# rkhosrowshahi/MO-VAE

Hardware: AMD Instinct MI355X
Metric: training images/sec (higher is better)
Workload: dtype f32

## Files before the change

include/movae.h:

```cpp
#ifndef MOVAE_H
#define MOVAE_H

#include <stddef.h>
#include <stdint.h>

#ifdef __cplusplus
extern "C" {
#endif

typedef void* movae_stream_t;

enum movae_act { MOVAE_ACT_NONE = 0, MOVAE_ACT_LRELU = 1, MOVAE_ACT_RELU = 2, MOVAE_ACT_TANH = 3, MOVAE_ACT_SIGMOID = 4 };
enum movae_recon { MOVAE_RECON_MSE = 0, MOVAE_RECON_BCE = 1, MOVAE_RECON_L1 = 2, MOVAE_RECON_SMOOTH_L1 = 3 };
enum movae_mgda_norm { MOVAE_MGDA_NONE = 0, MOVAE_MGDA_L2 = 1, MOVAE_MGDA_LOSS = 2, MOVAE_MGDA_LOSS_PLUS = 3 };
enum movae_upgrad_norm { MOVAE_UPGRAD_TRACE = 0, MOVAE_UPGRAD_MIN_L2 = 1, MOVAE_UPGRAD_COSINE = 2 };
enum movae_amtl_scale { MOVAE_AMTL_MIN = 0, MOVAE_AMTL_MEDIAN = 1, MOVAE_AMTL_RMSE = 2 };

int movae_version(void);
const char* movae_last_error(void);

int movae_nchw_to_nhwc(const float* src, float* dst, int n, int c, int h, int w, movae_stream_t stream);
int movae_nhwc_to_nchw(const float* src, float* dst, int n, int c, int h, int w, movae_stream_t stream);

int movae_conv2d_fwd(const float* x, const float* w, const float* bias, float* y,
// ... 135 lines not shown
int movae_vq_nearest_fwd_mse(const float* x, const float* e, float* q, int64_t* idx, float* sse, int32_t* used_count, float* mse2,
                             int rows, int k, int d, void* ws, size_t ws_bytes, movae_stream_t stream);
size_t movae_vq_bwd_ws_bytes(int rows, int k, int d);
int movae_vq_bwd(const float* x, const float* q, const int64_t* idx, const float* dq, const float* gc, const float* ge,
                 float* dx, float* de, int rows, int k, int d, void* ws, size_t ws_bytes, movae_stream_t stream);

#define MOVAE_MAX_K 8
size_t movae_gram_ws_bytes(int k, size_t m);
int movae_gram(const float* J, size_t ldj, int k, size_t m, float* G, void* ws, size_t ws_bytes, movae_stream_t stream);
int movae_weights_upgrad(const float* G, int k, float norm_eps, float reg_eps, const float* pref, float* w, movae_stream_t stream);
int movae_weights_upgrad_norm(const float* G, int k, int norm_mode, float norm_eps, float reg_eps, const float* pref, float* w,
                              movae_stream_t stream);
int movae_gram_upgrad(const float* J, size_t ldj, int k, size_t m, float* G, int norm_mode, float norm_eps, float reg_eps,
                      const float* pref, float* w, int dual, void* ws, size_t ws_bytes, movae_stream_t stream);
int movae_weights_mgda(const float* G, int k, int norm, const float* losses, float epsilon, int max_iters,
                       float* w, int32_t* info, movae_stream_t stream);
int movae_weights_mgda_stable(const float* G, int k, int norm, const float* losses, float epsilon, int max_iters,
                              float min_eigenvalue, float* w, int32_t* info, movae_stream_t stream);
int movae_weights_amtl(const float* G, int k, int scale_mode, const float* pref, float* w, movae_stream_t stream);
int movae_weights_dualproj(const float* G, int k, float norm_eps, float reg_eps, const float* pref, float* w, movae_stream_t stream);
int movae_weights_pcgrad(const float* G, int k, const int32_t* perm, float* w, movae_stream_t stream);
int movae_weights_imtlg(const float* G, int k, float* w, movae_stream_t stream);
int movae_weights_cagrad(const float* G, int k, float c, float norm_eps, float* w, movae_stream_t stream);
int movae_weights_const(int k, float value, float* w, movae_stream_t stream);
int movae_combine(const float* J, size_t ldj, int k, size_t m, const float* w, float* g, int accumulate, movae_stream_t stream);
int movae_gd_similarity(const float* J, size_t ldj, int k, size_t m, const float* w, float* out,
                        void* ws, size_t ws_bytes, movae_stream_t stream);

int movae_adam_step(float* p, const float* g, float* m, float* v, size_t n, float lr, float beta1, float beta2,
                    float eps, float weight_decay, int decoupled_wd, int step, movae_stream_t stream);
int movae_adam_multi(int n_tensors, float* const* p, const float* const* g, float* const* m, float* const* v,
                     const size_t* numel, float lr, float beta1, float beta2, float eps, float weight_decay,
                     int decoupled_wd, int step, float* hyper_dev, movae_stream_t stream);
int movae_clip_grad_norm_multi(int n_tensors, float* const* g, const size_t* numel, float max_norm, float* total_sumsq_dev,
                               void* ws, size_t ws_bytes, movae_stream_t stream);
int movae_sumsq(const float* x, size_t n, float* out, void* ws, size_t ws_bytes, movae_stream_t stream);
int movae_scale_by_clip(float* g, size_t n, const float* sumsq_dev, float max_norm, movae_stream_t stream);

#define MOVAE_DTYPE_F32 0
#define MOVAE_DTYPE_BF16 1
int movae_set_compute_dtype(int dtype);

int movae_reduce_defer(int on);
int movae_reduce_flush(void);
int movae_reduce_defer_stats(long long* out3, int reset);
long long movae_reduce_defer_max_bytes(long long bytes);

int movae_bench_main_kernel_only(int on);
const char* movae_bench_last_kernel(void);
int movae_bench_force_split(int s);
int movae_bench_kgemm_bn_fin(int mode);
int movae_bench_force_kgemm(int mode);

typedef struct movae_fuse {
    const float* in_scale;
    const float* in_shift;
    float in_slope;
    float* stats;
    size_t stats_cap;
    int stats_parts;
    const float* bn_y;
    const float* bn_scale;
    const float* bn_shift;
    float bn_slope;
    float* bn_part;
    size_t bn_cap;
// ... 109 lines not shown
```

mo-vae_amd/_lib.py:

```python
import ctypes as C
import os
import threading

import torch

HERE = os.path.dirname(os.path.abspath(__file__))
LIB_PATH = os.path.join(HERE, "libmovae_hip.so")

ACT = {"none": 0, None: 0, "lrelu": 1, "relu": 2, "tanh": 3, "sigmoid": 4}
RECON = {"mse": 0, "bce": 1, "l1": 2, "smooth_l1": 3}
UPGRAD_NORM = {"trace": 0, "min_l2": 1, "cosine": 2}
EDGE_MATCH = {"mag": 0, "signed_mse": 1, "maxnorm": 2, "angle": 3, "masked": 4, "cosine": 5}
MGDA_NORM = {"none": 0, "l2": 1, "loss": 2, "loss+": 3}
AMTL_SCALE = {"min": 0, "median": 1, "rmse": 2}
MAX_K = 8

_p, _i, _f, _z, _l = C.c_void_p, C.c_int, C.c_float, C.c_size_t, C.c_long

class MovaeFuse(C.Structure):
    _fields_ = [("in_scale", C.c_void_p), ("in_shift", C.c_void_p), ("in_slope", C.c_float), ("stats", C.c_void_p),
                ("stats_cap", C.c_size_t), ("stats_parts", C.c_int),
                ("bn_y", C.c_void_p), ("bn_scale", C.c_void_p), ("bn_shift", C.c_void_p), ("bn_slope", C.c_float), ("bn_part", C.c_void_p),
                ("bn_cap", C.c_size_t), ("bn_ppg", C.c_int),
                ("ep_act_y", C.c_void_p), ("ep_act", C.c_int), ("ep_slope", C.c_float), ("ep_act_done", C.c_int),
# ... 51 lines not shown
    "movae_sphere_latents_fwd": ([_p, _p, _p, _p, _i, _f, _i, _p, _i, _i, _i, _f, _f, _f, _f, _f, _f] + [_p] * 6 + [_p], _i),
    "movae_sphere_latents_bwd": ([_p] * 9 + [_i, _i, _f, _p], _i),
    "movae_sphere_losses_ws_bytes": ([_z, _i], _z),
    "movae_sphere_losses_fwd": ([_p, _p, _p, _p, _z, _p, _p, _i, _i, _f, _f, _f, _f, _f, _p, _p, _z, _p], _i),
    "movae_sphere_losses_bwd": ([_p, _p, _p, _p, _z, _p, _p, _i, _i, _f, _f, _f, _f, _f] + [_p] * 8 + [_p], _i),
    "movae_tc_decomp_fwd": ([_p] * 7 + [_i, _i, _p, _z, _p], _i),
    "movae_tc_decomp_bwd": ([_p] * 10 + [_i, _i, _p], _i),
    "movae_edge_weights": ([_p, _p, _p, _i, _i, _i, _i, _p, _z, _p], _i),
    "movae_edge_weighted_mse_fwd": ([_p, _p, _p, _p, _p, _i, _i, _i, _i, _f, _p, _z, _p], _i),
    "movae_edge_weighted_mse_bwd": ([_p, _p, _p, _p, _p, _p, _i, _i, _i, _i, _f, _p], _i),
    "movae_edge_match_fwd": ([_p, _p, _p, _i, _i, _i, _i, _f, _i, _p, _p, _z, _p], _i),
    "movae_edge_match_bwd": ([_p, _p, _p, _p, _p, _p, _i, _i, _i, _i, _f, _i, _p, _p], _i),
    "movae_vq_nearest_fwd": ([_p] * 6 + [_i, _i, _i, _p, _z, _p], _i),
    "movae_vq_nearest_fwd_mse": ([_p] * 7 + [_i, _i, _i, _p, _z, _p], _i),
    "movae_vq_bwd_ws_bytes": ([_i, _i, _i], _z),
    "movae_vq_bwd": ([_p] * 8 + [_i, _i, _i, _p, _z, _p], _i),
    "movae_gram_ws_bytes": ([_i, _z], _z),
    "movae_gram": ([_p, _z, _i, _z, _p, _p, _z, _p], _i),
    "movae_weights_upgrad": ([_p, _i, _f, _f, _p, _p, _p], _i),
    "movae_weights_upgrad_norm": ([_p, _i, _i, _f, _f, _p, _p, _p], _i),
    "movae_gram_upgrad": ([_p, _z, _i, _z, _p, _i, _f, _f, _p, _p, _i, _p, _z, _p], _i),
    "movae_weights_mgda": ([_p, _i, _i, _p, _f, _i, _p, _p, _p], _i),
    "movae_weights_mgda_stable": ([_p, _i, _i, _p, _f, _i, _f, _p, _p, _p], _i),
    "movae_weights_amtl": ([_p, _i, _i, _p, _p, _p], _i),
    "movae_weights_dualproj": ([_p, _i, _f, _f, _p, _p, _p], _i),
    "movae_weights_pcgrad": ([_p, _i, _p, _p, _p], _i),
    "movae_weights_imtlg": ([_p, _i, _p, _p], _i),
    "movae_weights_cagrad": ([_p, _i, _f, _f, _p, _p], _i),
    "movae_weights_const": ([_i, _f, _p, _p], _i),
    "movae_combine": ([_p, _z, _i, _z, _p, _p, _i, _p], _i),
    "movae_gd_similarity": ([_p, _z, _i, _z, _p, _p, _p, _z, _p], _i),
    "movae_adam_step": ([_p, _p, _p, _p, _z, _f, _f, _f, _f, _f, _i, _i, _p], _i),
    "movae_adam_multi": ([_i, _p, _p, _p, _p, _p, _f, _f, _f, _f, _f, _i, _i, _p, _p], _i),
    "movae_clip_grad_norm_multi": ([_i, _p, _p, _f, _p, _p, _z, _p], _i),
    "movae_sumsq": ([_p, _z, _p, _p, _z, _p], _i),
    "movae_scale_by_clip": ([_p, _z, _p, _f, _p], _i),
    "movae_conv2d_fwd_f": (_conv_fwd + [_p], _i),
    "movae_convT2d_fwd_f": (_conv_fwd + [_p], _i),
    "movae_conv2d_wgrad_grouped_f": ([_i] + _conv_wgrad + [_p], _i),
    "movae_convT2d_wgrad_grouped_f": ([_i] + _conv_wgrad + [_p], _i),
    "movae_conv2d_dgrad_wgrad_grouped_f": ([_i, _p, _p, _p, _p, _p, _p] + [_i] * 11 + [_i, _p, _z, _p, _p], _i),
    "movae_convT2d_dgrad_wgrad_grouped_f": ([_i, _p, _p, _p, _p, _p, _p] + [_i] * 11 + [_i, _p, _z, _p, _p], _i),
    "movae_conv2d_dgrad_f": (_conv_dgrad + [_p, _i], _i),
    "movae_convT2d_dgrad_f": (_conv_dgrad + [_p, _i], _i),
    "movae_bn_bwd_finalize": ([_p, _z, _i, _i, _i, _i, _p, _p, _p, _p, _p, _p, _i, _p], _i),
    "movae_bn_bwd_apply": ([_p, _p, _p, _p, _f, _p, _p, _i, _z, _i, _p], _i),
    "movae_linear_pair_fwd": ([_p, _p, _p, _p, _p, _p, _p, _i, _i, _i, _p], _i),
    "movae_linear_pair_bwd": ([_i, _p, _p, _p, _p, _p, _p, _p, _p, _p, _p, _i, _i, _i, _p], _i),
    "movae_bn_bwd_finalize_apply": ([_p, _z, _i, _i, _z, _i, _p, _p, _p, _p, _p, _p, _i, _p, _p, _p, _p, _f, _p, _p], _i),
    "movae_bn_finalize": ([_p, _z, _i, _i, _i, _p, _p, _f, _f, _p, _p, _p, _p, _p, _p, _p, _p], _i),
    "movae_bn_stats": ([_p, _i, _i, _p, _z, _p, _p], _i),
    "movae_scale_shift_act": ([_p, _p, _p, _p, _z, _i, _f, _p], _i),
    "movae_embedding_fwd": ([_p, _p, _p, _z, _i, _i, _p], _i),
    "movae_embedding_bwd": ([_p, _p, _p, _i, _i, _i, _p, _z, _p], _i),
    "movae_gated_residual_fwd": ([_p, _p, _p, _p, _z, _p], _i),
    "movae_gated_residual_bwd": ([_p, _p, _p, _p, _p, _z, _p], _i),
    "movae_mul": ([_p, _p, _p, _z, _p], _i),
    "movae_cross_entropy_ws_bytes": ([_z], _z),
    "movae_cross_entropy_fwd": ([_p, _p, _p, _p, _z, _i, _p, _z, _p], _i),
    "movae_cross_entropy_bwd": ([_p, _p, _p, _p, _p, _z, _i, _p], _i),
    "movae_causal_attn_fwd": ([_p, _p, _p, _l, _p, _p, _i, _i, _i, _i, _f, C.c_ulonglong, C.c_ulonglong, _p], _i),
    "movae_causal_attn_ws_bytes": ([_i, _i, _i], _z),
    "movae_causal_attn_bwd": ([_p, _p, _p, _l, _p, _p, _p, _p, _p, _p, _i, _i, _i, _i, _f, C.c_ulonglong, C.c_ulonglong, _p, _z, _p], _i),
    "movae_causal_attn_dropout_mask": ([_p, _i, _i, _f, C.c_ulonglong, C.c_ulonglong, _p], _i),
    "movae_attn_fwd": ([_p, _p, _p, _l, _p, _p, _p, _p, _i, _i, _i, _i, _f, _p], _i),
    "movae_attn_ws_bytes": ([_i, _i, _i], _z),
# ... 150 lines not shown
```

mo-vae_amd/aggregation.py:

```python
import os

import torch
import torch.nn as tnn

from . import _lib as L


def _st(t):
    return L.stream_ptr(t.device)


def _check_matrix(J):
    if J.dim() != 2:
        raise ValueError(f"Parameter `matrix` should be a tensor of dimension 2. Found `matrix.shape = {tuple(J.shape)}`.")
    if J.shape[0] > L.MAX_K:
        raise ValueError(f"at most {L.MAX_K} objectives are supported on device, got {J.shape[0]}")
    L.require_gpu(J)
    if J.dtype != torch.float32 or J.stride(1) != 1:
        raise ValueError("the Jacobian must be fp32 with unit column stride")


FUSE_GRAM = os.environ.get("MOVAE_FUSE_GRAM", "1") != "0"


# ... 33 lines not shown


class Weighting(tnn.Module):

    def forward(self, gramian):
        raise NotImplementedError


class _FromJacobian(tnn.Module):

    def __init__(self, gramian_weighting):
        super().__init__()
        self.gramian_weighting = gramian_weighting

    def forward(self, J):
        gw = self.gramian_weighting
        fused = getattr(gw, "from_jacobian", None)
        if fused is not None and FUSE_GRAM and not gw._forward_hooks and not gw._forward_pre_hooks:
            self.last_gramian, w = fused(J)
            return w
        self.last_gramian = compute_gramian(J)
        return gw(self.last_gramian)


class GramianWeightedAggregator(tnn.Module):
    def __init__(self, gramian_weighting):
        super().__init__()
        self.gramian_weighting = gramian_weighting
        self.weighting = _FromJacobian(gramian_weighting)

    def forward(self, J):
        w = self.weighting(J)
        return combine(J, w)


class UPGradWeighting(Weighting):

    def __init__(self, pref_vector=None, norm_eps=1e-4, reg_eps=1e-4, norm="trace"):
        super().__init__()
        self.pref_vector, self.norm_eps, self.reg_eps, self.norm = pref_vector, norm_eps, reg_eps, norm

    def _mode(self):
        return self.norm

    def forward(self, G):
        k = G.shape[0]
        w = torch.empty(k, dtype=torch.float32, device=G.device)
        pref = _pref_tensor(self.pref_vector, G.device)
        L.call("movae_weights_upgrad_norm", G.data_ptr(), k, L.UPGRAD_NORM[self._mode()], float(self.norm_eps),
               float(self.reg_eps), L.ptr(pref), w.data_ptr(), _st(G))
        return w

    def from_jacobian(self, J):
        _check_matrix(J)
        k, m = J.shape
        G = torch.empty((k, k), dtype=torch.float32, device=J.device)
        w = torch.empty(k, dtype=torch.float32, device=J.device)
        pref = _pref_tensor(self.pref_vector, J.device)
        ws = L.workspace(J.device)
        L.call("movae_gram_upgrad", J.data_ptr(), J.stride(0) if k > 1 else max(J.stride(0), m), k, m, G.data_ptr(),
               L.UPGRAD_NORM[self._mode()], float(self.norm_eps), float(self.reg_eps), L.ptr(pref), w.data_ptr(), 0, ws.data_ptr(),
               ws.numel(), _st(J))
        return G, w


class _PNUPGradWeighting(UPGradWeighting):
# ... 340 lines not shown
```

mo-vae_amd/autojac.py:

```python
import os

import torch

from . import ops

BATCHED_VJP = os.environ.get("MOVAE_BATCHED_VJP", "1") != "0"


def _leaf_tensors(roots, excluded=()):
    stop = {t.grad_fn for t in excluded if t.grad_fn is not None}
    seen, leaves, stack = set(), [], [t.grad_fn for t in roots if t.grad_fn is not None]
    while stack:
        fn = stack.pop()
        if fn is None or fn in seen or fn in stop:
            continue
        seen.add(fn)
        var = getattr(fn, "variable", None)
        if var is not None:
            if var.requires_grad:
                leaves.append(var)
            continue
        stack.extend(nf for nf, _ in fn.next_functions)
    out, ids = [], set()
    for v in leaves:
        if id(v) not in ids:
            ids.add(id(v))
            out.append(v)
    return out


def _mem_flat(t):
    if t.dim() == 4 and not t.is_contiguous():
# ... 222 lines not shown
                                     for i in range(len(per[0])))
                    if not isinstance(outs, tuple):
                        outs = (outs,)
                    need = [i for i, nd in enumerate(fn.needs_input_grad) if nd]
                    live = [j for j, (nf, _) in enumerate(edges) if nf is not None]
                    if len(need) != len(live):
                        raise NotImplementedError("cannot align backward outputs with graph edges")
                    aligned = [None] * len(edges)
                    for j, i in zip(live, need):
                        aligned[j] = outs[i] if i < len(outs) else None
                    outs = tuple(aligned)
                else:
                    per = []
                    for g in range(G):
                        r = fn(*[_group(a, g) for a in args])
                        per.append(r if isinstance(r, tuple) else (r,))
                    outs = tuple(None if all(per[g][i] is None for g in range(G)) else _restack([per[g][i] for g in range(G)])
                                 for i in range(len(per[0])))
            for i, (nf, nr) in enumerate(edges):
                if nf is None:
                    continue
                o = outs[i] if outs is not None and i < len(outs) else None
                if o is not None:
                    o = _fit_groups(o, _expected_shape(nf, nr), G)
                    slot = pending.setdefault(nf, {})
                    slot[nr] = _accumulate_stacked(slot.get(nr), o, G)
                deps[nf] -= 1
                if deps[nf] == 0:
                    ready.append(nf)
    finally:
        ops.GRAD_SINK_ROWS = None


def _aggregate_into_grads(jb, aggregator):
    g = aggregator(jb.J)
    for p, off in zip(jb.params, jb.offsets):
        _accumulate(p, _view_like(g[off: off + p.numel()], p))
    return g


class _MtlState:
    __slots__ = ("jb", "feat_diff", "feat_grads", "shared_params", "aggregator", "task_params", "device")


def mtl_backward_begin(losses, features, aggregator, tasks_params=None, shared_params=None):
    losses, features = list(losses), list(features)
    if len(losses) == 0:
        raise ValueError("`losses` cannot be empty")
    if len(features) == 0:
        raise ValueError("`features` cannot be empty.")
    if shared_params is None:
        shared_params = _leaf_tensors(features)
    if tasks_params is None:
        tasks_params = [_leaf_tensors([l], excluded=features) for l in losses]
    if len(tasks_params) != len(losses):
        raise ValueError("`losses` and `tasks_params` should have the same size.")
    st = _MtlState()
    st.shared_params = list(shared_params)
    st.aggregator = aggregator
    st.jb = JacobianBuffer.persistent(st.shared_params, len(losses), features[0].device)
    st.feat_diff = [f for f in features if f.requires_grad]
    st.feat_grads = []
    st.task_params = []
    cot = [torch.empty_strided((len(losses),) + tuple(f.shape), (f.numel(),) + tuple(f.stride()), dtype=f.dtype, device=f.device)
           if _dense(f) else None for f in st.feat_diff]
    for i, (loss, tp) in enumerate(zip(losses, tasks_params)):
        tp = list(tp)
        seed = _ones_like(loss) if loss.dim() == 0 and loss.dtype == torch.float32 else None
# ... 132 lines not shown
```

mo-vae_amd/csrc/agg.hip:

```cpp
#include "common.h"
#include <stdlib.h>

namespace {

constexpr int MAXK = MOVAE_MAX_K;
inline int gram_blocks(size_t m) {
    static const size_t cap = (size_t)env_long("MOVAE_GRAM_BLOCKS", 1024);
    size_t g = (m + 2047) / 2048;
    return (int)(g > cap ? cap : (g < 1 ? 1 : g));
}

template <int K, bool VEC>
__global__ __launch_bounds__(256) void gram_partial(const float* __restrict__ J, long ldj, long m, double* __restrict__ part) {
    constexpr int NP = K * (K + 1) / 2;
    double acc[NP];
#pragma unroll
    for (int q = 0; q < NP; ++q) acc[q] = 0.0;
    const long stride = (long)gridDim.x * blockDim.x;
    if (VEC) {
        const long nv = m / 4;
        for (long c = (long)blockIdx.x * blockDim.x + threadIdx.x; c < nv; c += stride) {
            f32x4 v[K];
#pragma unroll
            for (int i = 0; i < K; ++i) v[i] = reinterpret_cast<const f32x4*>(J + i * ldj)[c];
// ... 32 lines not shown
        if (threadIdx.x == 0) part[(long)blockIdx.x * NP + q] = s;
    }
}

__global__ __launch_bounds__(64) void gram_final(const double* __restrict__ part, int nblk, int K, float* __restrict__ G) {
    const int NP = K * (K + 1) / 2;
    const int q = blockIdx.x;
    double s = 0.0;
    for (int b = threadIdx.x; b < nblk; b += 64) s += part[(long)b * NP + q];
    s = wave_sum(s);
    if (threadIdx.x != 0) return;
    int i = 0, rem = q;
    while (rem >= K - i) {
        rem -= K - i;
        ++i;
    }
    const int j = i + rem;
    G[i * K + j] = (float)s;
    G[j * K + i] = (float)s;
}

template <int K, bool VEC>
__global__ __launch_bounds__(256) void combine_k(const float* __restrict__ J, long ldj, long m, const float* __restrict__ w,
                                                 float* __restrict__ g, int accumulate) {
    float wv[K];
#pragma unroll
    for (int i = 0; i < K; ++i) wv[i] = w[i];
    const long stride = (long)gridDim.x * blockDim.x;
    if (VEC) {
        const long nv = m / 4;
        for (long c = (long)blockIdx.x * blockDim.x + threadIdx.x; c < nv; c += stride) {
            f32x4 s = accumulate ? reinterpret_cast<const f32x4*>(g)[c] : f32x4{0.f, 0.f, 0.f, 0.f};
#pragma unroll
            for (int i = 0; i < K; ++i) s += wv[i] * reinterpret_cast<const f32x4*>(J + i * ldj)[c];
            reinterpret_cast<f32x4*>(g)[c] = s;
        }
        if (blockIdx.x == 0 && threadIdx.x == 0)
            for (long c = nv * 4; c < m; ++c) {
                float s = accumulate ? g[c] : 0.f;
                for (int i = 0; i < K; ++i) s += wv[i] * J[i * ldj + c];
                g[c] = s;
            }
    } else {
        for (long c = (long)blockIdx.x * blockDim.x + threadIdx.x; c < m; c += stride) {
            float s = accumulate ? g[c] : 0.f;
#pragma unroll
            for (int i = 0; i < K; ++i) s += wv[i] * J[i * ldj + c];
            g[c] = s;
        }
    }
}

__global__ __launch_bounds__(256) void similarity_partial(const float* __restrict__ J, long ldj, int K, long m,
                                                          const float* __restrict__ w, double* __restrict__ part) {
    __shared__ double sh[4];
    double ab = 0.0, aa = 0.0, bb = 0.0;
    const long stride = (long)gridDim.x * blockDim.x;
    for (long c = (long)blockIdx.x * blockDim.x + threadIdx.x; c < m; c += stride) {
        float a = 0.f, b = 0.f;
        for (int i = 0; i < K; ++i) {
            const float v = J[i * ldj + c];
            a += w[i] * v;
            b += v;
        }
        b /= (float)K;
        ab += (double)a * b;
        aa += (double)a * a;
        bb += (double)b * b;
    }
    ab = block_sum_256(ab, sh);
    aa = block_sum_256(aa, sh);
    bb = block_sum_256(bb, sh);
    if (threadIdx.x == 0) {
        part[blockIdx.x * 3 + 0] = ab;
        part[blockIdx.x * 3 + 1] = aa;
        part[blockIdx.x * 3 + 2] = bb;
    }
}

__global__ void similarity_final(const double* __restrict__ part, int nblk, float* __restrict__ out) {
// ... 741 lines not shown
```

mo-vae_amd/csrc/common.h:

```cpp
#pragma once
#include <hip/hip_runtime.h>
#include <stdint.h>
#include <stddef.h>
#include <stdio.h>
#include <stdlib.h>

#include "../../include/movae.h"

#define MOVAE_OK 0
#define MOVAE_EINVAL (-1)
#define MOVAE_EUNSUPPORTED (-2)
#define MOVAE_ELAUNCH (-3)

void movae_set_error(const char* fmt, ...);

#define MOVAE_CHECK_ARG(cond, ...)            \
    do {                                      \
        if (!(cond)) {                        \
            movae_set_error(__VA_ARGS__);     \
            return MOVAE_EINVAL;              \
        }                                     \
    } while (0)

#define MOVAE_CHECK_LAUNCH(name)                                                     \
// ... 99 lines not shown
        if (lane < CQB)
#pragma unroll
            for (int q = 0; q < NV; ++q) sh[q * 256 + wave * 64 + lane] = v[q];
        __syncthreads();
        if (t < CQB)
#pragma unroll
            for (int q = 0; q < NV; ++q)
                v[q] = (sh[q * 256 + t] + sh[q * 256 + 64 + t]) + (sh[q * 256 + 128 + t] + sh[q * 256 + 192 + t]);
    } else {
#pragma unroll
        for (int q = 0; q < NV; ++q) sh[q * 256 + t] = v[q];
        __syncthreads();
        if (t < CQB) {
            const int RG = 256 / CQB;
#pragma unroll
            for (int q = 0; q < NV; ++q) {
                double s = v[q];
                for (int i = 1; i < RG; ++i) s += sh[q * 256 + i * CQB + t];
                v[q] = s;
            }
        }
    }
    __syncthreads();
}

__device__ __forceinline__ double block_sum_256(double v, double* sh ) {
    v = wave_sum(v);
    const int w = threadIdx.x >> 6;
    __syncthreads();
    if ((threadIdx.x & 63) == 0) sh[w] = v;
    __syncthreads();
    return sh[0] + sh[1] + sh[2] + sh[3];
}
```

mo-vae_amd/csrc/optim.hip:

```cpp
#include "common.h"

namespace {

__global__ __launch_bounds__(256) void adam_k(float* __restrict__ p, const float* __restrict__ g, float* __restrict__ m,
                                              float* __restrict__ v, long n, float lr, float b1, float b2, float eps,
                                              float wd, int decoupled, float bc1, float bc2_sqrt) {
    const long stride = (long)gridDim.x * blockDim.x;
    for (long i = (long)blockIdx.x * blockDim.x + threadIdx.x; i < n; i += stride) {
        float gi = g[i], pi = p[i];
        if (wd != 0.f) {
            if (decoupled) pi *= 1.f - lr * wd;
            else gi += wd * pi;
        }
        const float mi = m[i] + (gi - m[i]) * (1.f - b1);
        const float vi = v[i] * b2 + (1.f - b2) * gi * gi;
        m[i] = mi;
        v[i] = vi;
        const float denom = sqrtf(vi) / bc2_sqrt + eps;
        p[i] = pi - (lr / bc1) * (mi / denom);
    }
}

constexpr int ADAM_MT = 64;
struct AdamTable {
    float* p[ADAM_MT];
    const float* g[ADAM_MT];
    float* m[ADAM_MT];
    float* v[ADAM_MT];
    unsigned n[ADAM_MT];
    unsigned first[ADAM_MT + 1];
};
constexpr unsigned ADAM_BLK = 4096;

__device__ __forceinline__ void adam_one(float& pi, float gi, float& mi, float& vi, float lr, float b1, float b2, float eps,
                                         float wd, int decoupled, float step_size, float bc2_sqrt) {
    if (wd != 0.f) {
        if (decoupled) pi *= 1.f - lr * wd;
        else gi += wd * pi;
    }
    mi = mi + (gi - mi) * (1.f - b1);
    vi = vi * b2 + (1.f - b2) * gi * gi;
    const float denom = sqrtf(vi) / bc2_sqrt + eps;
    pi = pi - step_size * (mi / denom);
}

__device__ unsigned g_adam_done = 0;

__global__ __launch_bounds__(256) void adam_multi_k(AdamTable tab, int cnt, float lr, float b1, float b2, float eps, float wd,
                                                    int decoupled, float bc1, float bc2_sqrt, float* __restrict__ hyper, int tick) {
    int t = 0;
    while (t + 1 < cnt && blockIdx.x >= tab.first[t + 1]) ++t;
    const unsigned n = tab.n[t], base = (blockIdx.x - tab.first[t]) * ADAM_BLK;
    float step_f = 0.f;
    if (hyper) {
        step_f = hyper[0] + 1.f;
        const double step = (double)step_f;
        lr = hyper[1];
        bc1 = (float)(1.0 - pow((double)b1, step));
        bc2_sqrt = (float)sqrt(1.0 - pow((double)b2, step));
    }
    const float step_size = lr / bc1;
    float* __restrict__ p = tab.p[t];
    const float* __restrict__ g = tab.g[t];
    float* __restrict__ m = tab.m[t];
    float* __restrict__ v = tab.v[t];
    const bool vec = ((reinterpret_cast<uintptr_t>(p) | reinterpret_cast<uintptr_t>(g) | reinterpret_cast<uintptr_t>(m) |
                       reinterpret_cast<uintptr_t>(v)) & 15) == 0;
    if (vec && base + ADAM_BLK <= n) {
        f32x4 pv[4], mv[4], vv[4], gv[4];
#pragma unroll
        for (int u = 0; u < 4; ++u) {
            const unsigned i = base + u * 1024u + threadIdx.x * 4;
            pv[u] = *reinterpret_cast<f32x4*>(p + i), mv[u] = *reinterpret_cast<f32x4*>(m + i), vv[u] = *reinterpret_cast<f32x4*>(v + i);
            gv[u] = *reinterpret_cast<const f32x4*>(g + i);
        }
#pragma unroll
        for (int u = 0; u < 4; ++u) {
            const unsigned i = base + u * 1024u + threadIdx.x * 4;
#pragma unroll
            for (int j = 0; j < 4; ++j) {
                float pj = pv[u][j], mj = mv[u][j], vj = vv[u][j];
                adam_one(pj, gv[u][j], mj, vj, lr, b1, b2, eps, wd, decoupled, step_size, bc2_sqrt);
                pv[u][j] = pj; mv[u][j] = mj; vv[u][j] = vj;
            }
            *reinterpret_cast<f32x4*>(p + i) = pv[u];
            *reinterpret_cast<f32x4*>(m + i) = mv[u];
            *reinterpret_cast<f32x4*>(v + i) = vv[u];
        }
    } else
    for (unsigned u = 0; u < 4; ++u) {
        const unsigned i = base + u * 1024u + threadIdx.x * 4;
        if (i >= n) break;
        if (vec && i + 4 <= n) {
            f32x4 pv = *reinterpret_cast<f32x4*>(p + i), mv = *reinterpret_cast<f32x4*>(m + i), vv = *reinterpret_cast<f32x4*>(v + i);
            const f32x4 gv = *reinterpret_cast<const f32x4*>(g + i);
#pragma unroll
            for (int j = 0; j < 4; ++j) {
                float pj = pv[j], mj = mv[j], vj = vv[j];
                adam_one(pj, gv[j], mj, vj, lr, b1, b2, eps, wd, decoupled, step_size, bc2_sqrt);
                pv[j] = pj; mv[j] = mj; vv[j] = vj;
            }
            *reinterpret_cast<f32x4*>(p + i) = pv;
            *reinterpret_cast<f32x4*>(m + i) = mv;
            *reinterpret_cast<f32x4*>(v + i) = vv;
        } else {
            const unsigned e = min(i + 4, n);
            for (unsigned k = i; k < e; ++k) {
                float pj = p[k], mj = m[k], vj = v[k];
                adam_one(pj, g[k], mj, vj, lr, b1, b2, eps, wd, decoupled, step_size, bc2_sqrt);
                p[k] = pj; m[k] = mj; v[k] = vj;
            }
        }
    }
    if (hyper) {
        __syncthreads();
        if (threadIdx.x == 0) {
            const unsigned done = atomicAdd(&g_adam_done, 1u);
            if (done == gridDim.x - 1) {
                g_adam_done = 0;
                if (tick) hyper[0] = step_f;
            }
        }
    }
}

__global__ __launch_bounds__(256) void sumsq_partial(const float* __restrict__ x, long n, double* __restrict__ part) {
    __shared__ double sh[4];
    double s = 0.0;
    const long stride = (long)gridDim.x * blockDim.x;
    for (long i = (long)blockIdx.x * blockDim.x + threadIdx.x; i < n; i += stride) s += (double)x[i] * x[i];
    s = block_sum_256(s, sh);
    if (threadIdx.x == 0) part[blockIdx.x] = s;
}

__global__ __launch_bounds__(256) void sumsq_final(const double* __restrict__ part, int nblk, float* __restrict__ out) {
    __shared__ double sh[4];
    double s = 0.0;
    for (int i = threadIdx.x; i < nblk; i += 256) s += part[i];
    s = block_sum_256(s, sh);
    if (threadIdx.x == 0) out[0] = (float)s;
}

// ... 24 lines not shown
    double s = 0.0;
    for (int i = threadIdx.x; i < nparts; i += 256) s += part[i];
    s = block_sum_256(s, sh);
    if (threadIdx.x == 0) sumsq[0] = accumulate ? sumsq[0] + (float)s : (float)s;
}

__global__ __launch_bounds__(256) void clip_multi_k(ClipTable tab, const float* __restrict__ sumsq, float max_norm) {
    const float coef = fminf(max_norm / (sqrtf(sumsq[0]) + 1e-6f), 1.f);
    if (coef >= 1.f) return;
    float* __restrict__ g = tab.g[blockIdx.y];
    const unsigned n = tab.n[blockIdx.y];
    for (unsigned i = blockIdx.x * 256u + threadIdx.x; i < n; i += gridDim.x * 256u) g[i] *= coef;
}

inline int blocks_for(size_t n) {
    size_t b = (n + 1023) / 1024;
    return (int)(b > 2048 ? 2048 : (b < 1 ? 1 : b));
}

}

extern "C" {

int movae_adam_step(float* p, const float* g, float* m, float* v, size_t n, float lr, float beta1, float beta2, float eps,
                    float weight_decay, int decoupled_wd, int step, movae_stream_t stream) {
    MOVAE_CHECK_ARG(p && g && m && v && n > 0 && step >= 1, "movae_adam_step: bad argument");
    const double bc1 = 1.0 - pow((double)beta1, step), bc2 = 1.0 - pow((double)beta2, step);
    hipLaunchKernelGGL(adam_k, dim3(blocks_for(n)), dim3(256), 0, (hipStream_t)stream, p, g, m, v, (long)n, lr, beta1, beta2, eps,
                       weight_decay, decoupled_wd, (float)bc1, (float)sqrt(bc2));
    MOVAE_CHECK_LAUNCH("adam");
    return MOVAE_OK;
}

int movae_adam_multi(int n_tensors, float* const* p, const float* const* g, float* const* m, float* const* v, const size_t* numel,
                     float lr, float beta1, float beta2, float eps, float weight_decay, int decoupled_wd, int step,
                     float* hyper_dev, movae_stream_t stream) {
    MOVAE_CHECK_ARG(n_tensors >= 0 && (n_tensors == 0 || (p && g && m && v && numel)), "movae_adam_multi: null table");
    MOVAE_CHECK_ARG(hyper_dev || step >= 1, "movae_adam_multi: step must be >= 1 when no device counter is given");
    float bc1 = 1.f, bc2_sqrt = 1.f;
    if (!hyper_dev) {
        bc1 = (float)(1.0 - pow((double)beta1, step));
        bc2_sqrt = (float)sqrt(1.0 - pow((double)beta2, step));
    }
    for (int t0 = 0; t0 < n_tensors; t0 += ADAM_MT) {
        AdamTable tab;
        const int cnt = n_tensors - t0 < ADAM_MT ? n_tensors - t0 : ADAM_MT;
        unsigned nblk = 0;
        for (int i = 0; i < cnt; ++i) {
            MOVAE_CHECK_ARG(p[t0 + i] && g[t0 + i] && m[t0 + i] && v[t0 + i], "movae_adam_multi: null tensor");
            MOVAE_CHECK_ARG(numel[t0 + i] > 0 && numel[t0 + i] < 0xffffffffUL, "movae_adam_multi: tensor size out of range");
            tab.p[i] = p[t0 + i]; tab.g[i] = g[t0 + i]; tab.m[i] = m[t0 + i]; tab.v[i] = v[t0 + i];
            tab.n[i] = (unsigned)numel[t0 + i];
            tab.first[i] = nblk;
            nblk += (unsigned)((numel[t0 + i] + ADAM_BLK - 1) / ADAM_BLK);
        }
        for (int i = cnt; i < ADAM_MT; ++i) { tab.p[i] = nullptr; tab.g[i] = nullptr; tab.m[i] = nullptr; tab.v[i] = nullptr; tab.n[i] = 0; }
        for (int i = cnt; i <= ADAM_MT; ++i) tab.first[i] = nblk;
        hipLaunchKernelGGL(adam_multi_k, dim3(nblk), dim3(256), 0, (hipStream_t)stream, tab, cnt, lr, beta1, beta2, eps, weight_decay,
                           decoupled_wd, bc1, bc2_sqrt, hyper_dev, t0 + ADAM_MT >= n_tensors ? 1 : 0);
        MOVAE_CHECK_LAUNCH("adam_multi");
    }
    return MOVAE_OK;
}

int movae_clip_grad_norm_multi(int n_tensors, float* const* g, const size_t* numel, float max_norm, float* total_sumsq_dev, void* ws,
                               size_t ws_bytes, movae_stream_t stream) {
    MOVAE_WS_SCRATCH(ws, ws_bytes);
    MOVAE_CHECK_ARG(n_tensors >= 1 && g && numel && total_sumsq_dev && max_norm > 0.f, "movae_clip_grad_norm_multi: bad argument");
    constexpr int BX = 32;
    MOVAE_CHECK_ARG(ws && ws_bytes >= (size_t)ADAM_MT * BX * sizeof(double), "movae_clip_grad_norm_multi: workspace too small");
    double* part = static_cast<double*>(ws);
    hipStream_t st = (hipStream_t)stream;
    for (int pass = 0; pass < 2; ++pass)
        for (int t0 = 0; t0 < n_tensors; t0 += ADAM_MT) {
            ClipTable tab;
            const int cnt = n_tensors - t0 < ADAM_MT ? n_tensors - t0 : ADAM_MT;
            for (int i = 0; i < ADAM_MT; ++i) {
                tab.g[i] = i < cnt ? g[t0 + i] : nullptr;
                tab.n[i] = i < cnt ? (unsigned)numel[t0 + i] : 0;
                if (i < cnt) MOVAE_CHECK_ARG(g[t0 + i] && numel[t0 + i] < 0xffffffffUL, "movae_clip_grad_norm_multi: bad tensor");
            }
            if (pass == 0) {
                hipLaunchKernelGGL(sumsq_multi_k, dim3(BX, cnt), dim3(256), 0, st, tab, part);
                MOVAE_CHECK_LAUNCH("sumsq_multi");
                hipLaunchKernelGGL(sumsq_multi_final, dim3(1), dim3(256), 0, st, part, BX * cnt, total_sumsq_dev, t0 > 0 ? 1 : 0);
                MOVAE_CHECK_LAUNCH("sumsq_multi_final");
            } else {
                hipLaunchKernelGGL(clip_multi_k, dim3(BX, cnt), dim3(256), 0, st, tab, total_sumsq_dev, max_norm);
                MOVAE_CHECK_LAUNCH("clip_multi");
            }
        }
    return MOVAE_OK;
}

int movae_sumsq(const float* x, size_t n, float* out, void* ws, size_t ws_bytes, movae_stream_t stream) {
// ... 21 lines not shown
```

mo-vae_amd/optim.py:

```python
import ctypes as C

import torch

from . import _lib as L


def _dense(t):
    return t.is_contiguous() or (t.dim() == 4 and t.is_contiguous(memory_format=torch.channels_last))


def _layout_differs(a, p):
    return a.shape != p.shape or any(n > 1 and x != y for n, x, y in zip(p.shape, a.stride(), p.stride()))


class FusedAdam(torch.optim.Adam):

    def __init__(self, params, lr=1e-3, betas=(0.9, 0.999), eps=1e-8, weight_decay=0.0, decoupled_weight_decay=False,
                 device_step=False):
        super().__init__(params, lr=lr, betas=betas, eps=eps, weight_decay=weight_decay, foreach=False, capturable=False)
        self._decoupled = bool(decoupled_weight_decay)
        self._device_step = bool(device_step)
        self._hyper = {}
        self._hyper_lr = {}

    def _group_hyper(self, gi, group, device):
        h = self._hyper.get(gi)
        if h is None:
            h = torch.tensor([0.0, float(group["lr"])], dtype=torch.float32, device=device)
            self._hyper[gi] = h
            self._hyper_lr[gi] = float(group["lr"])
        return h

    def sync_hyper(self):
        for gi, group in enumerate(self.param_groups):
            h = self._hyper.get(gi)
            if h is not None and self._hyper_lr[gi] != float(group["lr"]):
                h[1].fill_(float(group["lr"]))
                self._hyper_lr[gi] = float(group["lr"])

    @torch.no_grad()
    def step(self, closure=None):
        loss = None
        if closure is not None:
            with torch.enable_grad():
                loss = closure()
        for gi, group in enumerate(self.param_groups):
            if group.get("amsgrad") or group.get("maximize"):
                raise NotImplementedError("FusedAdam: amsgrad / maximize are not part of the reference's configuration")
            beta1, beta2 = group["betas"]
            buckets = {}
            hyper = None
            for p in group["params"]:
                g = p.grad
                if g is None:
                    continue
                L.require_gpu(p)
                if g.is_sparse:
                    raise RuntimeError("Adam does not support sparse gradients")
                if p.dtype != torch.float32 or not _dense(p):
                    raise NotImplementedError("FusedAdam: parameters must be dense fp32 tensors")
                if g.dtype != p.dtype or _layout_differs(g, p):
                    g = torch.empty_like(p).copy_(g)
                st = self.state[p]
                if len(st) == 0:
                    if self._device_step:
                        hyper = self._group_hyper(gi, group, p.device)
                        st["step"] = hyper[0]
                    else:
                        st["step"] = torch.tensor(0.0, dtype=torch.float32)
                    st["exp_avg"] = torch.zeros_like(p, memory_format=torch.preserve_format)
                    st["exp_avg_sq"] = torch.zeros_like(p, memory_format=torch.preserve_format)
                m, v = st["exp_avg"], st["exp_avg_sq"]
                if _layout_differs(m, p) or _layout_differs(v, p):
                    m = st["exp_avg"] = torch.empty_like(p).copy_(m)
                    v = st["exp_avg_sq"] = torch.empty_like(p).copy_(v)
                if self._device_step:
                    key = 0
                    if hyper is None:
                        hyper = self._group_hyper(gi, group, p.device)
                    if st["step"].data_ptr() != hyper.data_ptr():
                        hyper[0].copy_(st["step"])
                        st["step"] = hyper[0]
                else:
                    st["step"] += 1
                    key = int(st["step"].item())
                buckets.setdefault(key, []).append((p, g, m, v))
            for key, rows in buckets.items():
                n = len(rows)
                arr = C.c_void_p * n
                ps = arr(*[r[0].data_ptr() for r in rows])
                gs = arr(*[r[1].data_ptr() for r in rows])
                ms = arr(*[r[2].data_ptr() for r in rows])
                vs = arr(*[r[3].data_ptr() for r in rows])
                ns = (C.c_size_t * n)(*[r[0].numel() for r in rows])
                dev = rows[0][0].device
                if self._device_step and not torch.cuda.is_current_stream_capturing():
                    self.sync_hyper()
                L.call("movae_adam_multi", n, ps, gs, ms, vs, ns, float(group["lr"]), float(beta1), float(beta2),
                       float(group["eps"]), float(group["weight_decay"]), 1 if self._decoupled else 0,
                       max(1, key), L.ptr(hyper) if self._device_step else 0, L.stream_ptr(dev))
        return loss


class FusedAdamW(FusedAdam):

    def __init__(self, params, lr=1e-3, betas=(0.9, 0.999), eps=1e-8, weight_decay=1e-2, device_step=False):
        super().__init__(params, lr=lr, betas=betas, eps=eps, weight_decay=weight_decay, decoupled_weight_decay=True,
                         device_step=device_step)


def clip_grad_norm_(parameters, max_norm, norm_type=2.0):
    if float(norm_type) != 2.0:
        raise NotImplementedError("clip_grad_norm_: only the L2 norm of the reference's call is implemented")
    if isinstance(parameters, torch.Tensor):
        parameters = [parameters]
    grads = [p.grad for p in parameters if p.grad is not None]
    if not grads:
        return torch.tensor(0.0)
    for g in grads:
        L.require_gpu(g)
        if g.dtype != torch.float32 or not _dense(g):
            raise NotImplementedError("clip_grad_norm_: gradients must be dense fp32 tensors")
    dev = grads[0].device
    n = len(grads)
    sumsq = torch.empty((), dtype=torch.float32, device=dev)
    ws = L.workspace(dev)
    L.call("movae_clip_grad_norm_multi", n, (C.c_void_p * n)(*[g.data_ptr() for g in grads]),
           (C.c_size_t * n)(*[g.numel() for g in grads]), float(max_norm), sumsq.data_ptr(), ws.data_ptr(), ws.numel(),
           L.stream_ptr(dev))
    return sumsq.sqrt()
```

mo-vae_amd/train.py:

```python
import json
import math
import os
import time
from argparse import ArgumentParser

import torch
import torch.optim as optim

from . import _lib as L
from . import aggregation
from . import autojac
from . import ops
from .aggregation import COMFORT, MGDA
from .metrics import ReconMetricAccumulator, build_hv_indicator
from .models import get_network
from .optim import FusedAdam, FusedAdamW, clip_grad_norm_
from .parallel import DataParallelGrads

_current_step = 0
_hook_values = {}


class AverageMeter:

# ... 41 lines not shown
    optimizer.zero_grad()
    outputs = net(images)
    loss_dict = net.loss_function(images, args=outputs)
    if aggregator is None or aggregator == "sum":
        loss_dict["total_loss"].backward()
        return loss_dict, outputs, None
    features = [outputs[f] for f in net.features] if net.features is not None else None
    component_losses = [v for k, v in loss_dict.items() if k != "total_loss"]
    if isinstance(aggregator, (MGDA, COMFORT)):
        aggregator.set_losses(_stacked(component_losses))
    if features is None:
        if getattr(net, "_jacobian_from_loss_op", False):
            autojac.backward_through(component_losses, aggregator)
        else:
            autojac.backward(component_losses, aggregator=aggregator)
        return loss_dict, outputs, None
    pending = autojac.mtl_backward_begin(component_losses, features, aggregator)
    pending.device = images.device
    return loss_dict, outputs, pending


def forward_backward_finish(pending):
    if pending is not None:
        autojac.mtl_backward_finish(pending)


def forward_backward(net, images, optimizer, aggregator):
    loss_dict, outputs, pending = forward_backward_begin(net, images, optimizer, aggregator)
    forward_backward_finish(pending)
    return loss_dict, outputs


def train_step(net, images, optimizer, aggregator, args, dp=None):
    loss_dict, outputs = forward_backward(net, images, optimizer, aggregator)
    if dp is not None:
        dp.all_reduce_grads()
    if getattr(args, "max_grad_norm", None) is not None:
        clip_grad_norm_(net.parameters(), max_norm=args.max_grad_norm)
    optimizer.step()
    return loss_dict, outputs




DP_OVERLAP_MIN_BYTES = 32 << 20


def _state_tensors(net):
    extra = [t for t in (getattr(net, "_iter_dev", None), getattr(net, "_noise_state_t", None)) if isinstance(t, torch.Tensor)]
    return list(net.parameters()) + list(net.buffers()) + extra


def _snapshot_state(net, optimizer, device):
    return {"tensors": [t.detach().clone() for t in _state_tensors(net)],
            "opt": {id(p): {k: v.detach().clone() for k, v in st.items() if torch.is_tensor(v)} for p, st in optimizer.state.items()},
            "cuda_rng": torch.cuda.get_rng_state(device), "cpu_rng": torch.get_rng_state()}


@torch.no_grad()
def _restore_state(snap, net, optimizer, device):
    torch.cuda.synchronize(device)
    for t, s in zip(_state_tensors(net), snap["tensors"]):
        t.copy_(s)
    for p, st in optimizer.state.items():
        old = snap["opt"].get(id(p), {})
        for k, v in st.items():
            if torch.is_tensor(v):
# ... 626 lines not shown
```

Baseline: 338,300.

## Fold Jacobian weighted combine into the fused Adam step kernel

Instead of running a separate combine kernel that writes the aggregated gradient and then an Adam kernel that reads it back, the aggregator's weights are computed, and the combine is deferred to the optimizer. The fused Adam kernel then reads the K Jacobian rows, forms the gradient on the fly, writes it to .grad and applies the update, saving one kernel launch and one read of the gradient buffer. This applies only when there is no data parallelism or grad clipping. It adds bookkeeping and a fallback path that materializes the gradient if the layout checks fail.

```diff
diff --git a/include/movae.h b/include/movae.h
--- a/include/movae.h
+++ b/include/movae.h
@@ -191,6 +191,10 @@
 int movae_adam_multi(int n_tensors, float* const* p, const float* const* g, float* const* m, float* const* v,
                      const size_t* numel, float lr, float beta1, float beta2, float eps, float weight_decay,
                      int decoupled_wd, int step, float* hyper_dev, movae_stream_t stream);
+int movae_adam_multi_combined(int n_tensors, float* const* p, float* const* g, float* const* m, float* const* v,
+                              const size_t* numel, const long long* joff, const float* J, size_t ldj, int k, size_t jcols,
+                              const float* w, float lr, float beta1, float beta2, float eps, float weight_decay,
+                              int decoupled_wd, int step, float* hyper_dev, movae_stream_t stream);
 int movae_clip_grad_norm_multi(int n_tensors, float* const* g, const size_t* numel, float max_norm, float* total_sumsq_dev,
                                void* ws, size_t ws_bytes, movae_stream_t stream);
 int movae_sumsq(const float* x, size_t n, float* out, void* ws, size_t ws_bytes, movae_stream_t stream);
diff --git a/mo-vae_amd/_lib.py b/mo-vae_amd/_lib.py
--- a/mo-vae_amd/_lib.py
+++ b/mo-vae_amd/_lib.py
@@ -107,6 +107,7 @@
     "movae_gd_similarity": ([_p, _z, _i, _z, _p, _p, _p, _z, _p], _i),
     "movae_adam_step": ([_p, _p, _p, _p, _z, _f, _f, _f, _f, _f, _i, _i, _p], _i),
     "movae_adam_multi": ([_i, _p, _p, _p, _p, _p, _f, _f, _f, _f, _f, _i, _i, _p, _p], _i),
+    "movae_adam_multi_combined": ([_i, _p, _p, _p, _p, _p, _p, _p, _z, _i, _z, _p, _f, _f, _f, _f, _f, _i, _i, _p, _p], _i),
     "movae_clip_grad_norm_multi": ([_i, _p, _p, _f, _p, _p, _z, _p], _i),
     "movae_sumsq": ([_p, _z, _p, _p, _z, _p], _i),
     "movae_scale_by_clip": ([_p, _z, _p, _f, _p], _i),
diff --git a/mo-vae_amd/aggregation.py b/mo-vae_amd/aggregation.py
--- a/mo-vae_amd/aggregation.py
+++ b/mo-vae_amd/aggregation.py
@@ -89,6 +89,13 @@
     def forward(self, J):
         w = self.weighting(J)
         return combine(J, w)
+
+
+def weights_only(aggregator, J):
+    if (isinstance(aggregator, GramianWeightedAggregator) and type(aggregator).forward is GramianWeightedAggregator.forward
+            and not aggregator._forward_hooks and not aggregator._forward_pre_hooks):
+        return aggregator.weighting(J)
+    return None
 
 
 class UPGradWeighting(Weighting):
diff --git a/mo-vae_amd/autojac.py b/mo-vae_amd/autojac.py
--- a/mo-vae_amd/autojac.py
+++ b/mo-vae_amd/autojac.py
@@ -1,3 +1,4 @@
+import contextlib
 import os
 
 import torch
@@ -286,8 +287,25 @@
         ops.GRAD_SINK_ROWS = None
 
 
+_COMBINE_INTO = [None]
+
+
+@contextlib.contextmanager
+def combine_into(optimizer):
+    prev, _COMBINE_INTO[0] = _COMBINE_INTO[0], optimizer
+    try:
+        yield
+    finally:
+        _COMBINE_INTO[0] = prev
+
+
 def _aggregate_into_grads(jb, aggregator):
-    g = aggregator(jb.J)
+    opt, w = _COMBINE_INTO[0], None
+    if opt is not None and all(p.grad is None for p in jb.params):
+        from . import aggregation
+
+        w = aggregation.weights_only(aggregator, jb.J)
+    g = opt.defer_combine(jb.J, w, jb.params, jb.offsets) if w is not None else aggregator(jb.J)
     for p, off in zip(jb.params, jb.offsets):
         _accumulate(p, _view_like(g[off: off + p.numel()], p))
     return g
diff --git a/mo-vae_amd/csrc/agg.hip b/mo-vae_amd/csrc/agg.hip
--- a/mo-vae_amd/csrc/agg.hip
+++ b/mo-vae_amd/csrc/agg.hip
@@ -88,20 +88,20 @@
         for (long c = (long)blockIdx.x * blockDim.x + threadIdx.x; c < nv; c += stride) {
             f32x4 s = accumulate ? reinterpret_cast<const f32x4*>(g)[c] : f32x4{0.f, 0.f, 0.f, 0.f};
 #pragma unroll
-            for (int i = 0; i < K; ++i) s += wv[i] * reinterpret_cast<const f32x4*>(J + i * ldj)[c];
+            for (int i = 0; i < K; ++i) s = combine_term(s, wv[i], reinterpret_cast<const f32x4*>(J + i * ldj)[c]);
             reinterpret_cast<f32x4*>(g)[c] = s;
         }
         if (blockIdx.x == 0 && threadIdx.x == 0)
             for (long c = nv * 4; c < m; ++c) {
                 float s = accumulate ? g[c] : 0.f;
-                for (int i = 0; i < K; ++i) s += wv[i] * J[i * ldj + c];
+                for (int i = 0; i < K; ++i) s = combine_term(s, wv[i], J[i * ldj + c]);
                 g[c] = s;
             }
     } else {
         for (long c = (long)blockIdx.x * blockDim.x + threadIdx.x; c < m; c += stride) {
             float s = accumulate ? g[c] : 0.f;
 #pragma unroll
-            for (int i = 0; i < K; ++i) s += wv[i] * J[i * ldj + c];
+            for (int i = 0; i < K; ++i) s = combine_term(s, wv[i], J[i * ldj + c]);
             g[c] = s;
         }
     }
diff --git a/mo-vae_amd/csrc/common.h b/mo-vae_amd/csrc/common.h
--- a/mo-vae_amd/csrc/common.h
+++ b/mo-vae_amd/csrc/common.h
@@ -155,3 +155,8 @@
     __syncthreads();
     return sh[0] + sh[1] + sh[2] + sh[3];
 }
+
+template <class T>
+__device__ __forceinline__ T combine_term(T s, float w, T j) {
+    return s + w * j;
+}
diff --git a/mo-vae_amd/csrc/optim.hip b/mo-vae_amd/csrc/optim.hip
--- a/mo-vae_amd/csrc/optim.hip
+++ b/mo-vae_amd/csrc/optim.hip
@@ -1,4 +1,5 @@
 #include "common.h"
+#include <type_traits>
 
 namespace {
 
@@ -44,10 +45,48 @@
     pi = pi - step_size * (mi / denom);
 }
 
+struct AdamComb {
+    const float* J;
+    const float* w;
+    long ldj;
+    int K;
+    long off[ADAM_MT];
+};
+struct AdamNoComb {};
+
+__device__ __forceinline__ f32x4 adam_grad4(const float* __restrict__ g, const float* __restrict__ Jt, long ldj, int K,
+                                            const float (&wv)[MOVAE_MAX_K], bool jvec, unsigned i) {
+    if (!Jt) return *reinterpret_cast<const f32x4*>(g + i);
+    f32x4 s = {0.f, 0.f, 0.f, 0.f};
+#pragma unroll
+    for (int k = 0; k < MOVAE_MAX_K; ++k)
+        if (k < K) {
+            const float* r = Jt + k * ldj + i;
+            f32x4 j;
+            if (jvec) j = *reinterpret_cast<const f32x4*>(r);
+            else j = f32x4{r[0], r[1], r[2], r[3]};
+            s = combine_term(s, wv[k], j);
+        }
+    *reinterpret_cast<f32x4*>(const_cast<float*>(g) + i) = s;
+    return s;
+}
+__device__ __forceinline__ float adam_grad1(const float* __restrict__ g, const float* __restrict__ Jt, long ldj, int K,
+                                            const float (&wv)[MOVAE_MAX_K], unsigned i) {
+    if (!Jt) return g[i];
+    float s = 0.f;
+#pragma unroll
+    for (int k = 0; k < MOVAE_MAX_K; ++k)
+        if (k < K) s = combine_term(s, wv[k], Jt[k * ldj + i]);
+    const_cast<float*>(g)[i] = s;
+    return s;
+}
+
 __device__ unsigned g_adam_done = 0;
 
-__global__ __launch_bounds__(256) void adam_multi_k(AdamTable tab, int cnt, float lr, float b1, float b2, float eps, float wd,
+template <class CB>
+__global__ __launch_bounds__(256) void adam_multi_k(AdamTable tab, CB cb, int cnt, float lr, float b1, float b2, float eps, float wd,
                                                     int decoupled, float bc1, float bc2_sqrt, float* __restrict__ hyper, int tick) {
+    constexpr bool COMB = std::is_same<CB, AdamComb>::value;
     int t = 0;
     while (t + 1 < cnt && blockIdx.x >= tab.first[t + 1]) ++t;
     const unsigned n = tab.n[t], base = (blockIdx.x - tab.first[t]) * ADAM_BLK;
@@ -64,6 +103,20 @@
     const float* __restrict__ g = tab.g[t];
     float* __restrict__ m = tab.m[t];
     float* __restrict__ v = tab.v[t];
+    const float* Jt = nullptr;
+    long ldj = 0;
+    int K = 0;
+    float wv[MOVAE_MAX_K] = {};
+    bool jvec = false;
+    if constexpr (COMB) {
+        if (cb.off[t] >= 0) {
+            Jt = cb.J + cb.off[t], ldj = cb.ldj, K = cb.K;
+#pragma unroll
+            for (int k = 0; k < MOVAE_MAX_K; ++k)
+                if (k < K) wv[k] = cb.w[k];
+            jvec = (reinterpret_cast<uintptr_t>(Jt) & 15) == 0 && (ldj & 3) == 0;
+        }
+    }
     const bool vec = ((reinterpret_cast<uintptr_t>(p) | reinterpret_cast<uintptr_t>(g) | reinterpret_cast<uintptr_t>(m) |
                        reinterpret_cast<uintptr_t>(v)) & 15) == 0;
     if (vec && base + ADAM_BLK <= n) {
@@ -72,7 +125,7 @@
         for (int u = 0; u < 4; ++u) {
             const unsigned i = base + u * 1024u + threadIdx.x * 4;
             pv[u] = *reinterpret_cast<f32x4*>(p + i), mv[u] = *reinterpret_cast<f32x4*>(m + i), vv[u] = *reinterpret_cast<f32x4*>(v + i);
-            gv[u] = *reinterpret_cast<const f32x4*>(g + i);
+            gv[u] = adam_grad4(g, Jt, ldj, K, wv, jvec, i);
         }
 #pragma unroll
         for (int u = 0; u < 4; ++u) {
@@ -93,7 +146,7 @@
         if (i >= n) break;
         if (vec && i + 4 <= n) {
             f32x4 pv = *reinterpret_cast<f32x4*>(p + i), mv = *reinterpret_cast<f32x4*>(m + i), vv = *reinterpret_cast<f32x4*>(v + i);
-            const f32x4 gv = *reinterpret_cast<const f32x4*>(g + i);
+            const f32x4 gv = adam_grad4(g, Jt, ldj, K, wv, jvec, i);
 #pragma unroll
             for (int j = 0; j < 4; ++j) {
                 float pj = pv[j], mj = mv[j], vj = vv[j];
@@ -107,7 +160,7 @@
             const unsigned e = min(i + 4, n);
             for (unsigned k = i; k < e; ++k) {
                 float pj = p[k], mj = m[k], vj = v[k];
-                adam_one(pj, g[k], mj, vj, lr, b1, b2, eps, wd, decoupled, step_size, bc2_sqrt);
+                adam_one(pj, adam_grad1(g, Jt, ldj, K, wv, k), mj, vj, lr, b1, b2, eps, wd, decoupled, step_size, bc2_sqrt);
                 p[k] = pj; m[k] = mj; v[k] = vj;
             }
         }
@@ -198,11 +251,12 @@
     return MOVAE_OK;
 }
 
-int movae_adam_multi(int n_tensors, float* const* p, const float* const* g, float* const* m, float* const* v, const size_t* numel,
-                     float lr, float beta1, float beta2, float eps, float weight_decay, int decoupled_wd, int step,
-                     float* hyper_dev, movae_stream_t stream) {
-    MOVAE_CHECK_ARG(n_tensors >= 0 && (n_tensors == 0 || (p && g && m && v && numel)), "movae_adam_multi: null table");
-    MOVAE_CHECK_ARG(hyper_dev || step >= 1, "movae_adam_multi: step must be >= 1 when no device counter is given");
+static int adam_multi_launch(const char* who, int n_tensors, float* const* p, const float* const* g, float* const* m, float* const* v,
+                             const size_t* numel, const long long* joff, const AdamComb* comb, size_t jcols, float lr, float beta1,
+                             float beta2, float eps, float weight_decay, int decoupled_wd, int step, float* hyper_dev,
+                             movae_stream_t stream) {
+    MOVAE_CHECK_ARG(n_tensors >= 0 && (n_tensors == 0 || (p && g && m && v && numel)), "%s: null table", who);
+    MOVAE_CHECK_ARG(hyper_dev || step >= 1, "%s: step must be >= 1 when no device counter is given", who);
     float bc1 = 1.f, bc2_sqrt = 1.f;
     if (!hyper_dev) {
         bc1 = (float)(1.0 - pow((double)beta1, step));
@@ -210,23 +264,54 @@
     }
     for (int t0 = 0; t0 < n_tensors; t0 += ADAM_MT) {
         AdamTable tab;
+        AdamComb cb{};
+        if (comb) cb = *comb;
         const int cnt = n_tensors - t0 < ADAM_MT ? n_tensors - t0 : ADAM_MT;
         unsigned nblk = 0;
         for (int i = 0; i < cnt; ++i) {
-            MOVAE_CHECK_ARG(p[t0 + i] && g[t0 + i] && m[t0 + i] && v[t0 + i], "movae_adam_multi: null tensor");
-            MOVAE_CHECK_ARG(numel[t0 + i] > 0 && numel[t0 + i] < 0xffffffffUL, "movae_adam_multi: tensor size out of range");
+            MOVAE_CHECK_ARG(p[t0 + i] && g[t0 + i] && m[t0 + i] && v[t0 + i], "%s: null tensor", who);
+            MOVAE_CHECK_ARG(numel[t0 + i] > 0 && numel[t0 + i] < 0xffffffffUL, "%s: tensor size out of range", who);
             tab.p[i] = p[t0 + i]; tab.g[i] = g[t0 + i]; tab.m[i] = m[t0 + i]; tab.v[i] = v[t0 + i];
             tab.n[i] = (unsigned)numel[t0 + i];
             tab.first[i] = nblk;
             nblk += (unsigned)((numel[t0 + i] + ADAM_BLK - 1) / ADAM_BLK);
-        }
-        for (int i = cnt; i < ADAM_MT; ++i) { tab.p[i] = nullptr; tab.g[i] = nullptr; tab.m[i] = nullptr; tab.v[i] = nullptr; tab.n[i] = 0; }
+            if (comb) {
+                const long long off = joff[t0 + i];
+                MOVAE_CHECK_ARG(off < 0 || (size_t)off + numel[t0 + i] <= jcols, "%s: tensor %d lies outside the Jacobian's columns", who, t0 + i);
+                cb.off[i] = off < 0 ? -1 : (long)off;
+            }
+        }
+        for (int i = cnt; i < ADAM_MT; ++i) { tab.p[i] = nullptr; tab.g[i] = nullptr; tab.m[i] = nullptr; tab.v[i] = nullptr; tab.n[i] = 0; cb.off[i] = -1; }
         for (int i = cnt; i <= ADAM_MT; ++i) tab.first[i] = nblk;
-        hipLaunchKernelGGL(adam_multi_k, dim3(nblk), dim3(256), 0, (hipStream_t)stream, tab, cnt, lr, beta1, beta2, eps, weight_decay,
-                           decoupled_wd, bc1, bc2_sqrt, hyper_dev, t0 + ADAM_MT >= n_tensors ? 1 : 0);
+        const int tick = t0 + ADAM_MT >= n_tensors ? 1 : 0;
+        if (comb)
+            hipLaunchKernelGGL(adam_multi_k<AdamComb>, dim3(nblk), dim3(256), 0, (hipStream_t)stream, tab, cb, cnt, lr, beta1, beta2, eps,
+                               weight_decay, decoupled_wd, bc1, bc2_sqrt, hyper_dev, tick);
+        else
+            hipLaunchKernelGGL(adam_multi_k<AdamNoComb>, dim3(nblk), dim3(256), 0, (hipStream_t)stream, tab, AdamNoComb{}, cnt, lr, beta1,
+                               beta2, eps, weight_decay, decoupled_wd, bc1, bc2_sqrt, hyper_dev, tick);
         MOVAE_CHECK_LAUNCH("adam_multi");
     }
     return MOVAE_OK;
+}
+
+int movae_adam_multi(int n_tensors, float* const* p, const float* const* g, float* const* m, float* const* v, const size_t* numel,
+                     float lr, float beta1, float beta2, float eps, float weight_decay, int decoupled_wd, int step,
+                     float* hyper_dev, movae_stream_t stream) {
+    return adam_multi_launch("movae_adam_multi", n_tensors, p, g, m, v, numel, nullptr, nullptr, 0, lr, beta1, beta2, eps, weight_decay,
+                             decoupled_wd, step, hyper_dev, stream);
+}
+
+int movae_adam_multi_combined(int n_tensors, float* const* p, float* const* g, float* const* m, float* const* v, const size_t* numel,
+                              const long long* joff, const float* J, size_t ldj, int k, size_t jcols, const float* w, float lr,
+                              float beta1, float beta2, float eps, float weight_decay, int decoupled_wd, int step, float* hyper_dev,
+                              movae_stream_t stream) {
+    MOVAE_CHECK_ARG(joff && J && w && jcols > 0 && ldj >= jcols, "movae_adam_multi_combined: bad Jacobian argument");
+    MOVAE_CHECK_ARG(k >= 1 && k <= MOVAE_MAX_K, "movae_adam_multi_combined: k=%d outside 1..%d", k, MOVAE_MAX_K);
+    AdamComb cb{};
+    cb.J = J, cb.w = w, cb.ldj = (long)ldj, cb.K = k;
+    return adam_multi_launch("movae_adam_multi_combined", n_tensors, p, g, m, v, numel, joff, &cb, jcols, lr, beta1, beta2, eps,
+                             weight_decay, decoupled_wd, step, hyper_dev, stream);
 }
 
 int movae_clip_grad_norm_multi(int n_tensors, float* const* g, const size_t* numel, float max_norm, float* total_sumsq_dev, void* ws,
diff --git a/mo-vae_amd/optim.py b/mo-vae_amd/optim.py
--- a/mo-vae_amd/optim.py
+++ b/mo-vae_amd/optim.py
@@ -13,6 +13,24 @@
     return a.shape != p.shape or any(n > 1 and x != y for n, x, y in zip(p.shape, a.stride(), p.stride()))
 
 
+class DeferredCombine:
+
+    def __init__(self, J, w, params, offsets):
+        self.J, self.w = J, w
+        self.g = torch.empty(J.shape[1], dtype=torch.float32, device=J.device)
+        self.params = list(params)
+        self.col = {id(p): off for p, off in zip(params, offsets)}
+
+    @property
+    def ldj(self):
+        k, m = self.J.shape
+        return self.J.stride(0) if k > 1 else max(self.J.stride(0), m)
+
+    def materialize(self):
+        k, m = self.J.shape
+        L.call("movae_combine", self.J.data_ptr(), self.ldj, k, m, self.w.data_ptr(), self.g.data_ptr(), 0, L.stream_ptr(self.J.device))
+
+
 class FusedAdam(torch.optim.Adam):
 
     def __init__(self, params, lr=1e-3, betas=(0.9, 0.999), eps=1e-8, weight_decay=0.0, decoupled_weight_decay=False,
@@ -22,6 +40,29 @@
         self._device_step = bool(device_step)
         self._hyper = {}
         self._hyper_lr = {}
+        self._deferred = None
+
+    def defer_combine(self, J, w, params, offsets):
+        self.flush_combine()
+        self._deferred = DeferredCombine(J, w, params, offsets)
+        return self._deferred.g
+
+    def flush_combine(self):
+        d, self._deferred = self._deferred, None
+        if d is not None:
+            d.materialize()
+
+    def _take_deferred(self):
+        d, self._deferred = self._deferred, None
+        if d is None:
+            return None
+        mine = {id(p) for group in self.param_groups for p in group["params"]}
+        ok = all(id(p) in mine and p.grad is not None and p.grad.dtype == torch.float32 and p.dtype == torch.float32 and _dense(p)
+                 and p.grad.data_ptr() == d.g.data_ptr() + 4 * d.col[id(p)] and not _layout_differs(p.grad, p) for p in d.params)
+        if not ok:
+            d.materialize()
+            return None
+        return d
 
     def _group_hyper(self, gi, group, device):
         h = self._hyper.get(gi)
@@ -44,6 +85,7 @@
         if closure is not None:
             with torch.enable_grad():
                 loss = closure()
+        comb = self._take_deferred()
         for gi, group in enumerate(self.param_groups):
             if group.get("amsgrad") or group.get("maximize"):
                 raise NotImplementedError("FusedAdam: amsgrad / maximize are not part of the reference's configuration")
@@ -84,7 +126,7 @@
                 else:
                     st["step"] += 1
                     key = int(st["step"].item())
-                buckets.setdefault(key, []).append((p, g, m, v))
+                buckets.setdefault(key, []).append((p, g, m, v, comb.col.get(id(p), -1) if comb is not None else -1))
             for key, rows in buckets.items():
                 n = len(rows)
                 arr = C.c_void_p * n
@@ -96,9 +138,14 @@
                 dev = rows[0][0].device
                 if self._device_step and not torch.cuda.is_current_stream_capturing():
                     self.sync_hyper()
-                L.call("movae_adam_multi", n, ps, gs, ms, vs, ns, float(group["lr"]), float(beta1), float(beta2),
-                       float(group["eps"]), float(group["weight_decay"]), 1 if self._decoupled else 0,
-                       max(1, key), L.ptr(hyper) if self._device_step else 0, L.stream_ptr(dev))
+                tail = (float(group["lr"]), float(beta1), float(beta2), float(group["eps"]), float(group["weight_decay"]),
+                        1 if self._decoupled else 0, max(1, key), L.ptr(hyper) if self._device_step else 0, L.stream_ptr(dev))
+                if comb is not None and any(r[4] >= 0 for r in rows):
+                    k, jcols = comb.J.shape
+                    L.call("movae_adam_multi_combined", n, ps, gs, ms, vs, ns, (C.c_longlong * n)(*[r[4] for r in rows]),
+                           comb.J.data_ptr(), comb.ldj, k, jcols, comb.w.data_ptr(), *tail)
+                else:
+                    L.call("movae_adam_multi", n, ps, gs, ms, vs, ns, *tail)
         return loss
 
 
diff --git a/mo-vae_amd/train.py b/mo-vae_amd/train.py
--- a/mo-vae_amd/train.py
+++ b/mo-vae_amd/train.py
@@ -97,7 +97,9 @@
 
 
 def train_step(net, images, optimizer, aggregator, args, dp=None):
-    loss_dict, outputs = forward_backward(net, images, optimizer, aggregator)
+    fold = dp is None and getattr(args, "max_grad_norm", None) is None and hasattr(optimizer, "defer_combine")
+    with autojac.combine_into(optimizer if fold else None):
+        loss_dict, outputs = forward_backward(net, images, optimizer, aggregator)
     if dp is not None:
         dp.all_reduce_grads()
     if getattr(args, "max_grad_norm", None) is not None:
```

Result: no change. 335,800 (median of 2 runs) (-0.7%).
